# SciML/NeuralPDE.jl

Hardware: NVIDIA H100
Metric: collocation-points/sec (loss+grad) (higher is better)
Workload: dtype f32

## Files before the change

neuralpde.jl_b200/csrc/tc_kernel.cu:

```cuda
#include "tc_common.cuh"

namespace pinn {

using Fp = FpBlock<kTcW>;

struct CtaShared : CtaBase {
  int split, off_Q;
  uint8_t* stash;
  TcNetSmem nets[PINN_MAX_NETS];
};

struct LoopCtx {
  uint32_t fp;
  uint32_t bt;
  uint32_t tP;
  uint32_t tQ;
  float* gb;
  float* gw;
  uint32_t taddr;
  int act, split, p, lane, g0, g1, flag;
  __device__ __forceinline__ LoopCtx(uint32_t fp_, uint32_t bt_, uint32_t tP_, uint32_t tQ_, const Tid& t, int act_, int ng,
                                     int flag_, int split_ = 0, float* gb_ = nullptr, float* gw_ = nullptr)
      : fp(fp_), bt(bt_), tP(tP_), tQ(tQ_), gb(gb_), gw(gw_), taddr(t.lane_addr), act(act_), split(split_), p(t.p), lane(t.lane),
        g0(t.hh * (ng / kNH)), g1((t.hh + 1) * (ng / kNH)), flag(flag_) {}
};

template <int N1, int N2, bool PURE, int AK>
__device__ __forceinline__ void l0_fwd_loop(const LoopCtx lc, const PassInfo<N1, N2> pi, const float* xp, float* up) {
  constexpr int C = 1 + N1 + N2;
  float x[PINN_MAX_IN], u[C];
#pragma unroll
  for (int k = 0; k < PINN_MAX_IN; ++k) x[k] = xp[k];
#pragma unroll
  for (int c = 0; c < C; ++c) u[c] = up[c];
#pragma unroll 1
  for (int g = lc.g0; g < lc.g1; ++g) {
    float h[C][GW];
#pragma unroll
    for (int i = 0; i < GW; i += 2) {
      float za[C], zb2[C];
      first_layer_elem<kTcW>(lc.fp, pi, x, g * GW + i, za);
      first_layer_elem<kTcW>(lc.fp, pi, x, g * GW + i + 1, zb2);
      P2 zz[C], hv[C];
#pragma unroll
      for (int c = 0; c < C; ++c) zz[c] = mk2(za[c], zb2[c]);
      chain_fwd<N1, N2, PURE, AK, P2>(lc.act, pi.ch, zz, hv);
#pragma unroll
      for (int c = 0; c < C; ++c) { h[c][i] = hv[c].v.x; h[c][i + 1] = hv[c].v.y; }
      if (lc.flag) {
        const float w0 = lds_f32(lc.fp + (Fp::WL + g * GW + i) * 4), w1 = lds_f32(lc.fp + (Fp::WL + g * GW + i + 1) * 4);
#pragma unroll
        for (int c = 0; c < C; ++c) u[c] = fmaf(w1, hv[c].v.y, fmaf(w0, hv[c].v.x, u[c]));
      }
    }
#pragma unroll
    for (int c = 0; c < C; ++c) store_half(lc.tP + c * kTileBytes, lc.tQ + c * kTileBytes, lc.p, g * GW, h[c], lc.split != 0);
  }
#pragma unroll
  for (int c = 0; c < C; ++c) up[c] = u[c];
}

template <int C, int NK, bool SPLIT>
__device__ __forceinline__ void fwd_mma(float (&d)[C][16], uint32_t sP, uint32_t sQ, uint32_t whi, uint32_t wlo) {
  const int wg = threadIdx.x >> 7;
  const uint32_t aoff = (wg & 1) * 8192u, boff = (wg >> 1) * 32u * 128u;
  const uint64_t dwhi = tc::make_desc(whi + boff, 0, 1024), dwlo = tc::make_desc(wlo + boff, 0, 1024);
  tc::wgmma_fence();
#pragma unroll
  for (int c = 0; c < C; ++c) {
    const uint64_t dahi = tc::make_desc(sP + c * kTileBytes + aoff, 0, 1024);
    const uint64_t dalo = tc::make_desc(sQ + c * kTileBytes + aoff, 0, 1024);
#pragma unroll
    for (int pr = 0; pr < (SPLIT ? 3 : 1); ++pr) {
      const uint64_t a = (pr == 2) ? dalo : dahi, b = (pr == 1) ? dwlo : dwhi;
#pragma unroll
      for (int k = 0; k < NK; ++k)
        tc::wgmma_n32<0, 0>(d[c], a + 2 * k, b + 2 * k, (pr | k) ? 1u : 0u);
    }
  }
  tc::wgmma_commit();
  tc::wgmma_wait0();
}
template <int C>
__device__ __forceinline__ void fwd_mma_any(float (&d)[C][16], uint32_t sP, uint32_t sQ, uint32_t whi, uint32_t wlo, int nk,
                                            bool split) {
  switch (nk * 2 + (split ? 1 : 0)) {
    case 2: fwd_mma<C, 1, false>(d, sP, sQ, whi, wlo); break;
    case 3: fwd_mma<C, 1, true>(d, sP, sQ, whi, wlo); break;
    case 4: fwd_mma<C, 2, false>(d, sP, sQ, whi, wlo); break;
    case 5: fwd_mma<C, 2, true>(d, sP, sQ, whi, wlo); break;
    case 6: fwd_mma<C, 3, false>(d, sP, sQ, whi, wlo); break;
    case 7: fwd_mma<C, 3, true>(d, sP, sQ, whi, wlo); break;
    case 8: fwd_mma<C, 4, false>(d, sP, sQ, whi, wlo); break;
    default: fwd_mma<C, 4, true>(d, sP, sQ, whi, wlo); break;
  }
}

template <int N1, int N2, bool PURE, int AK, int C>
__device__ __forceinline__ void tl_fwd_frag(const float (&d)[C][16], const LoopCtx lc, const Chan<N1, N2> ch, float* scratch) {
  const int wg = threadIdx.x >> 7, w = (threadIdx.x >> 5) & 3;
  const int row0 = 64 * (wg & 1) + 16 * w + (lc.lane >> 2);
  const int col0 = 32 * (wg >> 1) + 2 * (lc.lane & 3);
  float u[2][C];
#pragma unroll
  for (int r = 0; r < 2; ++r)
#pragma unroll
    for (int c = 0; c < C; ++c) u[r][c] = 0.f;
#pragma unroll
  for (int i = 0; i < 16; i += 2) {
    const int rh = (i >> 1) & 1;
    const int row = row0 + 8 * rh, col = col0 + 8 * (i >> 2);
    P2 zz[C], hv[C];
    zz[0] = mk2(d[0][i] + lds_f32(lc.bt + col * 4), d[0][i + 1] + lds_f32(lc.bt + (col + 1) * 4));
#pragma unroll
    for (int c = 1; c < C; ++c) zz[c] = mk2(d[c][i], d[c][i + 1]);
    chain_fwd<N1, N2, PURE, AK, P2>(lc.act, ch, zz, hv);
    const uint32_t off = tc::swz_off(row, col);
#pragma unroll
    for (int c = 0; c < C; ++c) {
      const uint32_t hx = tc::pack_bf16(hv[c].v.x, hv[c].v.y);
      asm volatile("st.shared.b32 [%0], %1;" ::"r"(lc.tP + c * kTileBytes + off), "r"(hx) : "memory");
      if (lc.split)
        asm volatile("st.shared.b32 [%0], %1;" ::"r"(lc.tQ + c * kTileBytes + off), "r"(bf16x2_lo(hv[c].v.x, hv[c].v.y, hx))
                     : "memory");
    }
    if (lc.flag) {
      const float w0 = lds_f32(lc.fp + (Fp::WL + col) * 4), w1 = lds_f32(lc.fp + (Fp::WL + col + 1) * 4);
#pragma unroll
      for (int c = 0; c < C; ++c) u[rh][c] = fmaf(w1, hv[c].v.y, fmaf(w0, hv[c].v.x, u[rh][c]));
    }
  }
  if (lc.flag) {
#pragma unroll
    for (int r = 0; r < 2; ++r)
#pragma unroll
      for (int c = 0; c < C; ++c) {
        float s = u[r][c];
        s += __shfl_xor_sync(0xffffffffu, s, 1);
        s += __shfl_xor_sync(0xffffffffu, s, 2);
        if ((lc.lane & 3) == 0) atomicAdd(&scratch[c * kTcPts + row0 + 8 * r], s);
      }
  }
}

template <int C, int NKO>
__device__ __forceinline__ void dgrad_mma(float (&d)[C][16], uint32_t sP, uint32_t whi) {
  const uint32_t poff = (threadIdx.x >> 7) * 32u * 128u;
  const uint64_t dw = tc::make_desc(whi, 0, 1024);
  tc::wgmma_fence();
#pragma unroll
  for (int c = 0; c < C; ++c) {
    const uint64_t dz = tc::make_desc(sP + c * kTileBytes + poff, 0, 1024);
#pragma unroll
    for (int k = 0; k < NKO; ++k)
      tc::wgmma_n32<1, 0>(d[c], dw + 128 * k, dz + 2 * k, k ? 1u : 0u);
  }
  tc::wgmma_commit();
  tc::wgmma_wait0();
}
template <int C>
__device__ __forceinline__ void dgrad_mma_any(float (&d)[C][16], uint32_t sP, uint32_t whi, int nko) {
  switch (nko) {
    case 1: dgrad_mma<C, 1>(d, sP, whi); break;
    case 2: dgrad_mma<C, 2>(d, sP, whi); break;
    case 3: dgrad_mma<C, 3>(d, sP, whi); break;
    default: dgrad_mma<C, 4>(d, sP, whi); break;
  }
}
template <int C>
__device__ __forceinline__ void wgrad_mma(float (&dw)[32], float (&db)[8], uint32_t sP, uint32_t sQ, uint32_t s_ones) {
  const uint32_t poff = (threadIdx.x >> 7) * 32u * 128u;
  const uint64_t d1 = tc::make_desc(s_ones, 0, 0);
  tc::wgmma_fence();
#pragma unroll
  for (int c = 0; c < C; ++c) {
    const uint64_t dh = tc::make_desc(sQ + c * kTileBytes + poff, 0, 1024), dz = tc::make_desc(sP + c * kTileBytes + poff, 0, 1024);
#pragma unroll
    for (int k = 0; k < 2; ++k) tc::wgmma_n64<1, 1>(dw, dh + 128 * k, dz + 128 * k, (c | k) ? 1u : 0u);
  }
  const uint64_t dz0 = tc::make_desc(sP + poff, 0, 1024);
#pragma unroll
  for (int k = 0; k < 2; ++k) tc::wgmma_n16<1, 1>(db, dz0 + 128 * k, d1, k ? 1u : 0u);
  tc::wgmma_commit();
  tc::wgmma_wait0();
}

template <int NF>
__device__ __forceinline__ void frag_store_rows(float* base, int ld, const float (&d)[NF]) {
  const int w = (threadIdx.x >> 5) & 3, lane = threadIdx.x & 31;
  const bool odd = (lane & 1) != 0;
  float* row = base + (16 * w + (lane >> 2) + (odd ? 8 : 0)) * ld + 4 * ((lane >> 1) & 1);
#pragma unroll
  for (int j = 0; j < NF / 4; ++j) {
    const float r0 = __shfl_xor_sync(0xffffffffu, odd ? d[4 * j] : d[4 * j + 2], 1);
    const float r1 = __shfl_xor_sync(0xffffffffu, odd ? d[4 * j + 1] : d[4 * j + 3], 1);
    *reinterpret_cast<float4*>(row + 8 * j) =
        odd ? make_float4(r0, r1, d[4 * j + 2], d[4 * j + 3]) : make_float4(d[4 * j], d[4 * j + 1], r0, r1);
  }
}

template <int N1, int N2, bool PURE, int AK, int C>
__device__ __forceinline__ void tl_bwd_frag(const float (&d)[C][16], const LoopCtx lc, const Chan<N1, N2> ch, const float* ubs) {
  const int wg = threadIdx.x >> 7, w = (threadIdx.x >> 5) & 3;
  const int row0 = 64 * (wg & 1) + 16 * w + (lc.lane >> 2);
  const int col0 = 32 * (wg >> 1) + 2 * (lc.lane & 3);
  const float* hbar = tc::s_acc + TM_X * kAccRows;
#pragma unroll
  for (int i = 0; i < 16; i += 2) {
    const int row = row0 + 8 * ((i >> 1) & 1), col = col0 + 8 * (i >> 2);
    P2 zz[C], hv[C], zv[C];
    zz[0] = mk2(d[0][i] + lds_f32(lc.bt + col * 4), d[0][i + 1] + lds_f32(lc.bt + (col + 1) * 4));
#pragma unroll
    for (int c = 1; c < C; ++c) zz[c] = mk2(d[c][i], d[c][i + 1]);
    if (lc.flag) {
      const float w0 = lds_f32(lc.fp + (Fp::WL + col) * 4), w1 = lds_f32(lc.fp + (Fp::WL + col + 1) * 4);
#pragma unroll
      for (int c = 0; c < C; ++c) {
        const float u = ubs[c * kTcPts + row];
        hv[c] = mk2(w0 * u, w1 * u);
      }
    } else {
#pragma unroll
      for (int c = 0; c < C; ++c) hv[c] = mk2(hbar[(c * 64 + col) * kAccRows + row], hbar[(c * 64 + col + 1) * kAccRows + row]);
    }
    chain_bwd<N1, N2, PURE, AK, P2>(lc.act, ch, zz, hv, zv);
    const uint32_t off = tc::swz_off(row, col);
#pragma unroll
    for (int c = 0; c < C; ++c)
      asm volatile("st.shared.b32 [%0], %1;" ::"r"(lc.tP + c * kTileBytes + off), "r"(tc::pack_bf16(zv[c].v.x, zv[c].v.y))
                   : "memory");
  }
}

template <int N1, int N2, bool PURE, int AK>
__device__ __forceinline__ void l0_bwd_store_loop(const LoopCtx lc, const PassInfo<N1, N2> pi, const float* xp) {
  constexpr int C = 1 + N1 + N2;
  float x[PINN_MAX_IN];
#pragma unroll
  for (int k = 0; k < PINN_MAX_IN; ++k) x[k] = xp[k];
#pragma unroll 1
  for (int g = lc.g0; g < lc.g1; ++g) {
    float hb[C][GWB];
#pragma unroll
    for (int c = 0; c < C; ++c) acc_ldg(lc.taddr + TM_X + c * 64 + g * GWB, hb[c]);
#pragma unroll
    for (int i = 0; i < GWB; i += 2) {
      float za[C], zb2[C];
      first_layer_elem<kTcW>(lc.fp, pi, x, g * GWB + i, za);
      first_layer_elem<kTcW>(lc.fp, pi, x, g * GWB + i + 1, zb2);
      P2 zz[C], hv[C], zv[C];
#pragma unroll
      for (int c = 0; c < C; ++c) { zz[c] = mk2(za[c], zb2[c]); hv[c] = mk2(hb[c][i], hb[c][i + 1]); }
      chain_bwd<N1, N2, PURE, AK, P2>(lc.act, pi.ch, zz, hv, zv);
#pragma unroll
      for (int c = 0; c <= N1; ++c) { hb[c][i] = zv[c].v.x; hb[c][i + 1] = zv[c].v.y; }
    }
#pragma unroll
    for (int c = 0; c <= N1; ++c) store_half(lc.tP + c * kTileBytes, lc.tP, lc.p, g * GWB, hb[c], false);
  }
}

template <int N1, int N2, bool PURE, int AK>
__device__ __forceinline__ void l0_bwd_loop(const LoopCtx lc, const PassInfo<N1, N2> pi, const float* xp, const float* ubp) {
  constexpr int C = 1 + N1 + N2;
  float x[PINN_MAX_IN], ub[C];
#pragma unroll
  for (int k = 0; k < PINN_MAX_IN; ++k) x[k] = xp[k];
#pragma unroll
  for (int c = 0; c < C; ++c) ub[c] = ubp[c];
  const int re = reduceg_elem(lc.lane);
  const bool rlead = reduceg_lead(lc.lane);
  const int n1w = pi.n1w;
#pragma unroll 1
  for (int g = lc.g0; g < lc.g1; ++g) {
    float hb[C][GW];
    if (!lc.flag) {
#pragma unroll
      for (int c = 0; c < C; ++c) acc_ldg(lc.taddr + TM_X + c * 64 + g * GW, hb[c]);
    } else {
#pragma unroll
      for (int i = 0; i < GW; ++i) {
        const float wl = lds_f32(lc.fp + (Fp::WL + g * GW + i) * 4);
#pragma unroll
        for (int c = 0; c < C; ++c) hb[c][i] = wl * ub[c];
      }
    }
    float zv0[GW], zvd[N1 > 0 ? N1 : 1][GW];
#pragma unroll
    for (int i = 0; i < GW; ++i) {
      float zz[C], hv[C], zv[C];
      first_layer_elem<kTcW>(lc.fp, pi, x, g * GW + i, zz);
#pragma unroll
      for (int c = 0; c < C; ++c) hv[c] = hb[c][i];
      chain_bwd<N1, N2, PURE, AK, float>(lc.act, pi.ch, zz, hv, zv);
      zv0[i] = zv[0];
#pragma unroll
      for (int jd = 0; jd < N1; ++jd) zvd[jd][i] = zv[1 + jd];
    }
    const float bs = warp_reduceg(zv0, lc.lane);
    if (rlead) atomicAdd(lc.gb + g * GW + re, bs);
#pragma unroll
    for (int k = 0; k < PINN_MAX_IN; ++k) {
      if (k < pi.d_in) {
        float gk[GW];
#pragma unroll
        for (int i = 0; i < GW; ++i) {
          float gg = zv0[i] * x[k];
#pragma unroll
          for (int jd = 0; jd < N1; ++jd) gg += (pi.dir1[jd] == k) ? zvd[jd][i] : 0.f;
          gk[i] = gg;
        }
        const float gs = warp_reduceg(gk, lc.lane);
        if (rlead) atomicAdd(lc.gw + g * GW + re + (long long)n1w * k, gs);
      }
    }
  }
}

template <int N1, int N2, bool PURE, int AK>
__device__ __noinline__ uint32_t net_forward(CtaShared* cs, const DevProblem* Pp, const DevTerm* tmp, int slot,
                                             int want_grad, uint32_t phase) {
  extern __shared__ __align__(1024) uint8_t smem[];
  constexpr int C = 1 + N1 + N2;
  const DevTerm& tm = *tmp;
  const int net_id = tm.used_net[slot];
  const DevNet& net = Pp->nets[net_id];
  const DevChan& dc = tm.chan[slot];
  const TcNetSmem ns = cs->nets[net_id];
  const float* fp = reinterpret_cast<const float*>(smem + ns.fp);
  uint8_t* tP = smem + cs->off_P;
  uint8_t* tQ = smem + cs->off_Q;
  const Misc ms = misc_of(smem + cs->off_misc, cs->mx_dim, cs->mx_taps);
  const uint32_t accm = 0;
  const bool split = cs->split != 0;
  PassInfo<N1, N2> pi;
  load_pass<N1, N2>(pi, net, dc);
  const int TL = pi.TL;
  const Tid t = tid_of();
  const int tid = t.tid, p = t.p;
  float x[PINN_MAX_IN];
#pragma unroll
  for (int k = 0; k < PINN_MAX_IN; ++k) x[k] = (k < pi.d_in) ? ms.Xs[dc.rows[k] * kTcPts + p] : 0.f;
  uint8_t* stash_slot = cs->stash + (size_t)slot * cs->tl_max * kTcMaxC * kTileBytes;

  dbg_mark(cs, 10);
  float u[C];
#pragma unroll
  for (int c = 0; c < C; ++c) u[c] = 0.f;
  if (tid < C * kTcPts / 4) reinterpret_cast<float4*>(ms.scratch)[tid] = make_float4(0.f, 0.f, 0.f, 0.f);
  {
    const LoopCtx lc(tc::smem_u32(fp), tc::smem_u32(fp), tc::smem_u32(tP), tc::smem_u32(tQ), t, net.acts[0], pi.n1w / GW, TL == 0, split);
    l0_fwd_loop<N1, N2, PURE, AK>(lc, pi, x, u);
  }
  for (int l = 1; l <= TL; ++l) {
    const int n_in = net.dims[l], n_out = net.dims[l + 1];
    const int act = net.acts[l];
    tc::fence_async_smem();
    __syncthreads();
    dbg_mark(cs, 11);
    if (want_grad && tid == 0) {
      for (int c = 0; c < C; ++c)
        tc::bulk_store(stash_slot + (size_t)(l - 1) * kTcMaxC * kTileBytes + (size_t)c * kTileBytes, tP + c * kTileBytes, kTileBytes);
      tc::bulk_commit();
    }
    float d[C][16];
    {
      const uint32_t sP = tc::smem_u32(tP), sQ = tc::smem_u32(tQ);
      const uint32_t whi = tc::smem_u32(smem + ns.w_hi[l - 1]), wlo = tc::smem_u32(smem + ns.w_lo[l - 1]);
      const int nk = n_in / 16;
      fwd_mma_any<C>(d, sP, sQ, whi, wlo, nk, split);
    }
    dbg_mark(cs, 13);
    if (want_grad && tid == 0) tc::bulk_wait_read0();
    __syncthreads();
    dbg_mark(cs, 14);
    const LoopCtx lc(tc::smem_u32(fp), tc::smem_u32(fp) + (Fp::BT + (l - 1) * 64) * 4, tc::smem_u32(tP), tc::smem_u32(tQ), t, act, 0, l == TL, split);
    tl_fwd_frag<N1, N2, PURE, AK, C>(d, lc, pi.ch, ms.scratch);
  }
  finish_forward<C>(cs, tm, slot, ms, fp + Fp::BL, t, u);
  return phase;
}

template <int N1, int N2, bool PURE, int AK>
__device__ __noinline__ uint32_t net_backward(CtaShared* cs, const DevProblem* Pp, const DevTerm* tmp, int slot,
                                              uint32_t phase) {
  extern __shared__ __align__(1024) uint8_t smem[];
  constexpr int C = 1 + N1 + N2;
  const DevTerm& tm = *tmp;
  const int net_id = tm.used_net[slot];
  const DevNet& net = Pp->nets[net_id];
  const DevChan& dc = tm.chan[slot];
  const TcNetSmem ns = cs->nets[net_id];
  const float* fp = reinterpret_cast<const float*>(smem + ns.fp);
  uint8_t* tP = smem + cs->off_P;
  uint8_t* tQ = smem + cs->off_Q;
  const Misc ms = misc_of(smem + cs->off_misc, cs->mx_dim, cs->mx_taps);
  const uint32_t accm = 0;
  float* partial = cs->partial;
  PassInfo<N1, N2> pi;
  load_pass<N1, N2>(pi, net, dc);
  const int L = pi.L, TL = pi.TL;
  const Tid t = tid_of();
  const int tid = t.tid, p = t.p;
  uint32_t ld_phase = (phase >> 1) & 1u;
  float x[PINN_MAX_IN];
#pragma unroll
  for (int k = 0; k < PINN_MAX_IN; ++k) x[k] = (k < pi.d_in) ? ms.Xs[dc.rows[k] * kTcPts + p] : 0.f;
  uint8_t* stash_slot = cs->stash + (size_t)slot * cs->tl_max * kTcMaxC * kTileBytes;

  dbg_mark(cs, 20);
  float ub[C];
  gather_ubar<C>(tm, slot, ms, p, ub);
  if (t.hh == 0) {
#pragma unroll
    for (int c = 0; c < C; ++c) ms.scratch[c * kTcPts + p] = ub[c];
  }
  last_layer_grad<C>(t, ub, pi.nL, partial + net.w_off[L - 1], partial + net.b_off[L - 1], tc::smem_u32(tQ), tc::smem_u32(tP),
                     kTileBytes, 0u, accm + TM_Y, kTcW);

  const uint32_t sP = tc::smem_u32(tP), sQ = tc::smem_u32(tQ);
  const int wg = tid >> 7;
  float* hand = tc::s_acc + TM_X * kAccRows;
  float* wpart = reinterpret_cast<float*>(tP);
  float* bpart = ms.scratch;
  static_assert(4 * 64 <= kTcMaxC * kTcPts, "the bias partials fit ms.scratch");
  for (int l = TL; l >= 1; --l) {
    const int n_in = net.dims[l], n_out = net.dims[l + 1];
    const int act = net.acts[l];
    float* gb = partial + net.b_off[l];
    float* gw = partial + net.w_off[l];
    const float* bt = fp + Fp::BT + (l - 1) * 64;
    const uint32_t whi = tc::smem_u32(smem + ns.w_hi[l - 1]);
    dbg_mark(cs, 21);
    if (tid == 0 && l == TL) {
      const uint8_t* src = stash_slot + (size_t)(l - 1) * kTcMaxC * kTileBytes;
      tc::mbar_arrive_expect_tx(ms.bar_ld, C * kTileBytes);
      for (int c = 0; c < C; ++c) tc::bulk_load(tQ + c * kTileBytes, src + (size_t)c * kTileBytes, kTileBytes, ms.bar_ld);
    }
    wait_bar(ms.bar_ld, ld_phase);
    dbg_mark(cs, 22);
    {
      float d[C][16];
      fwd_mma_any<C>(d, sQ, sQ, whi, whi, n_in / 16, false);
      __syncthreads();
      dbg_mark(cs, 24);
      const LoopCtx lc(tc::smem_u32(fp), tc::smem_u32(bt), sP, sQ, t, act, 0, l == TL);
      tl_bwd_frag<N1, N2, PURE, AK, C>(d, lc, pi.ch, ms.scratch);
    }
    tc::fence_async_smem();
    __syncthreads();
    dbg_mark(cs, 26);
    {
      float d[C][16];
      dgrad_mma_any<C>(d, sP, whi, n_out / 16);
#pragma unroll
      for (int c = 0; c < C; ++c) frag_store_rows(hand + c * 64 * kAccRows + 32 * wg, kAccRows, d[c]);
    }
    dbg_mark(cs, 27);
    {
      float dw[32], db[8];
      wgrad_mma<C>(dw, db, sP, sQ, tc::smem_u32(smem + cs->off_ones));
      __syncthreads();
      if (tid == 0 && l > 1) {
        const uint8_t* src = stash_slot + (size_t)(l - 2) * kTcMaxC * kTileBytes;
        tc::mbar_arrive_expect_tx(ms.bar_ld, C * kTileBytes);
        for (int c = 0; c < C; ++c) tc::bulk_load(tQ + c * kTileBytes, src + (size_t)c * kTileBytes, kTileBytes, ms.bar_ld);
      }
      frag_store_rows(wpart + wg * 64 * 64, 64, dw);
      if ((t.lane & 3) == 0) {
        const int o = 16 * (t.warp & 3) + (t.lane >> 2);
        bpart[wg * 64 + o] = db[0];
        bpart[wg * 64 + o + 8] = db[2];
      }
    }
    __syncthreads();
    dbg_mark(cs, 28);
#pragma unroll 1
    for (int e = tid; e < 64 * 64; e += kTcThreads) {
      const int k = e >> 6, o = e & 63;
      if (k < n_in && o < n_out) atomicAdd(gw + o + (long long)n_out * k, ((wpart[e] + wpart[4096 + e]) + wpart[8192 + e]) + wpart[12288 + e]);
    }
    if (tid < n_out) atomicAdd(gb + tid, ((bpart[tid] + bpart[64 + tid]) + bpart[128 + tid]) + bpart[192 + tid]);
  }

  {
    __syncthreads();
    dbg_mark(cs, 29);
    const int act0 = net.acts[0];
    float* gb0 = partial + net.b_off[0];
    float* gw0 = partial + net.w_off[0];
    if (TL == 0) {
      const LoopCtx lc(tc::smem_u32(fp), tc::smem_u32(fp), sP, sQ, t, act0, pi.n1w / GW, 1, 0, gb0, gw0);
      l0_bwd_loop<N1, N2, PURE, AK>(lc, pi, x, ub);
    } else {
      coord_tiles<N1>(t, sQ, x, pi.dir1, N2 > 0);
      const LoopCtx lc(tc::smem_u32(fp), tc::smem_u32(fp), sP, sQ, t, act0, pi.n1w / GWB, 0);
      l0_bwd_store_loop<N1, N2, PURE, AK>(lc, pi, x);
      layer0_grad<N1>(t, sP, kTileBytes, 0u, sQ, N2 > 0, accm + TM_Y, kTcW, pi.n1w, pi.d_in, gw0, gb0);
    }
  }
  __syncthreads();
  dbg_mark(cs, 30);
  return (ld_phase << 1) | (phase & 1u);
}


__global__ void __launch_bounds__(kTcThreads, 1) tc_loss_grad_kernel(const __grid_constant__ TcArgs args) {
  extern __shared__ __align__(1024) uint8_t smem[];
  __shared__ CtaShared cs;
  const int tid = threadIdx.x;
  const DevProblem* Pp = args.prob;
  const DevProblem& P = *Pp;
  const Misc ms = misc_of(smem + args.off_misc, args.mx_dim, args.mx_taps);
  float* partial = args.partial + (long long)blockIdx.x * args.partial_stride;
  const bool want_grad = (args.mode == 0);
  const float* theta = args.theta;
  const DbgSpan span = dbg_span_begin(args.dbg);

  for (long long i = (long long)tid * 32; i < args.n_theta; i += (long long)kTcThreads * 32) tc::prefetch_l2(theta + i);
  {
    const char* nets0 = reinterpret_cast<const char*>(&Pp->nets[0]);
    const char* terms0 = reinterpret_cast<const char*>(&Pp->terms[0]);
    const int nb_nets = args.n_nets * (int)sizeof(DevNet), nb_terms = args.n_terms * (int)sizeof(DevTerm);
    if (tid == 0) tc::prefetch_l2(Pp);
    for (int o = tid * 128; o < nb_nets; o += kTcThreads * 128) tc::prefetch_l2(nets0 + o);
    for (int o = tid * 128; o < nb_terms; o += kTcThreads * 128) tc::prefetch_l2(terms0 + o);
    const int tile = args.tile_begin + (int)blockIdx.x;
    if (tile < args.tile_end && tid < 32) {
      int ti = 0;
      while (ti + 1 < args.n_terms && tile >= args.dyn[ti + 1].tile0) ++ti;
      const long long p0 = (long long)(tile - args.dyn[ti].tile0) * kTcPts;
      const long long row_bytes = 4ll * args.term_dim[ti];
      const long long off = p0 * row_bytes + (long long)tid * 128;
      if (off < args.dyn[ti].n * row_bytes) tc::prefetch_l2(reinterpret_cast<const char*>(args.dyn[ti].pts) + off);
    }
  }
  if (tid == 0) {
    tc::mbar_init(ms.bar_ld, 1);
    tc::fence_barrier_init();
    cs.split = args.split; cs.off_Q = args.off_Q;
    cs.stash = args.stash + (long long)blockIdx.x * args.stash_per_cta;
    for (int k = 0; k < PINN_MAX_NETS; ++k) cs.nets[k] = args.nets[k];
    cta_base_init(cs, args, partial);
  }
  if (tid == 0) tc::s_acc = args.acc + (size_t)blockIdx.x * kAccCols * kAccRows;
  cta_setup(args, ms, partial, P.n_theta, want_grad);
  for (int kn = 0; kn < P.n_nets; ++kn) {
    const DevNet& net = P.nets[kn];
    const TcNetSmem& ns = args.nets[kn];
    if (ns.fp < 0) continue;
    stage_fp_block<kTcW>(reinterpret_cast<float*>(smem + ns.fp), net, theta);
    const int L = net.n_layers;
    {
      constexpr int kItMax = kTcMaxTL * 512 / kTcThreads;
      const int n_items = (L - 2) * 512;
      float w[kItMax][8];
#pragma unroll
      for (int it = 0; it < kItMax; ++it) {
        const int i = tid + it * kTcThreads;
        if (i < n_items) {
          const int l = 1 + i / 512, r = i & 511;
          const int o = r & 63, kc = r >> 6;
          const int n_in = net.dims[l], n_out = net.dims[l + 1];
          const long long woff = net.w_off[l];
#pragma unroll
          for (int e = 0; e < 8; ++e) {
            const int k = kc * 8 + e;
            w[it][e] = (o < n_out && k < n_in) ? __ldg(&theta[woff + o + (long long)n_out * k]) : 0.f;
          }
        }
      }
#pragma unroll
      for (int it = 0; it < kItMax; ++it) {
        const int i = tid + it * kTcThreads;
        if (i < n_items) {
          const int l = 1 + i / 512, r = i & 511;
          const int o = r & 63, kc = r >> 6;
          uint8_t* thi = smem + ns.w_hi[l - 1];
          uint8_t* tlo = smem + ns.w_lo[l - 1];
          const float* v = w[it];
          uint32_t h[4];
#pragma unroll
          for (int e = 0; e < 4; ++e) h[e] = tc::pack_bf16(v[2 * e], v[2 * e + 1]);
          *reinterpret_cast<uint4*>(thi + tc::swz_chunk(o, kc)) = make_uint4(h[0], h[1], h[2], h[3]);
          if (args.split)
            *reinterpret_cast<uint4*>(tlo + tc::swz_chunk(o, kc)) = make_uint4(
                bf16x2_lo(v[0], v[1], h[0]), bf16x2_lo(v[2], v[3], h[1]), bf16x2_lo(v[4], v[5], h[2]), bf16x2_lo(v[6], v[7], h[3]));
        }
      }
    }
  }
  tc::fence_async_smem();
  __syncthreads();
  dbg_mark(&cs, 2);
  uint32_t phase = 0;

  for (int tile = args.tile_begin + blockIdx.x; tile < args.tile_end; tile += gridDim.x) {
    if (tid >= 128 && tid < 128 + (int)((sizeof(DevNet) * PINN_MAX_NETS + 127) / 128))
      tc::prefetch_l1(reinterpret_cast<const char*>(&P.nets[0]) + (tid - 128) * 128);
    uint32_t ldp = (phase >> 1) & 1u;
    const TileRef tr = stage_tile(args, P, ms, tile, ldp);
    phase = (phase & 1u) | (ldp << 1);
    const DevTerm* tmp = &P.terms[tr.ti];
    const DevTerm& tm = *tmp;
    const int n_used = tm.n_used;
    dbg_mark(&cs, 3);

    for (int slot = 0; slot < n_used; ++slot) {
      const int k1 = tm.chan[slot].n1, k2 = tm.chan[slot].n2, pu = tm.chan[slot].pure;
      const int ak = args.net_ak[tm.used_net[slot]];
      PINN_TC_DISPATCH(kTcMaxC, k1, k2, pu, ak, (phase = net_forward<A1, A2, PU, AK>(&cs, Pp, tmp, slot, want_grad ? 1 : 0, phase)));
    }

    dbg_mark(&cs, 4);
    residual_step(args, P, tm, ms, tr, smem + args.off_Q, (size_t)args.off_Q_bytes, partial, want_grad);

    dbg_mark(&cs, 5);
    if (want_grad) {
      if (tid == 0) tc::bulk_wait0();
      __syncthreads();
      dbg_mark(&cs, 6);
      for (int slot = n_used - 1; slot >= 0; --slot) {
        const int k1 = tm.chan[slot].n1, k2 = tm.chan[slot].n2, pu = tm.chan[slot].pure;
        const int ak = args.net_ak[tm.used_net[slot]];
        if (n_used > 1) {
          PINN_TC_DISPATCH(kTcMaxC, k1, k2, pu, ak, (phase = net_forward<A1, A2, PU, AK>(&cs, Pp, tmp, slot, 0, phase)));
        }
        PINN_TC_DISPATCH(kTcMaxC, k1, k2, pu, ak, (phase = net_backward<A1, A2, PU, AK>(&cs, Pp, tmp, slot, phase)));
      }
    }
  }

  __syncthreads();
  dbg_mark(&cs, 7);
  cta_finish(args, cs, span, ms, P, want_grad);
}

size_t tc_misc_bytes(int mx_dim, int mx_taps) {
  return (size_t)mx_dim * kTcPts * 4 + 2 * (size_t)mx_taps * kTcPts * 4 + (size_t)kTcMaxC * kTcPts * 4 + kTcPts * 4 +
         PINN_MAX_TERMS * 8 + 16 + 16;
}

cudaError_t tc_launch(const TcArgs& a, int grid, size_t smem, cudaStream_t st) {
  return launch_fused_kernel<tc_loss_grad_kernel>(a, grid, kTcThreads, smem, st);
}

}
```

Baseline: 94.15 million.

## Compute last-layer and layer-0 weight grads with wgmma, drop atomics for plain RMW

Replaces the previous last-layer and layer-0 gradient helpers with wgmma-based reductions over staged bf16 tiles. Per-warpgroup partials go through shared memory and are summed once per block. The per-layer atomicAdd loops on the block-private partial buffer become plain load-add-store, and L2 prefetches for the gradient slices are issued ahead of the updates. This removes atomic traffic and scalar reduction work, at the cost of extra __syncthreads, more shared-memory staging, and bf16 rounding of ub in the last-layer product.

New measurement: 96.44 million (median of 6 runs). Within noise of the previous version (+2.4%).

```diff
diff --git a/neuralpde.jl_b200/csrc/tc_kernel.cu b/neuralpde.jl_b200/csrc/tc_kernel.cu
--- a/neuralpde.jl_b200/csrc/tc_kernel.cu
+++ b/neuralpde.jl_b200/csrc/tc_kernel.cu
@@ -185,6 +185,54 @@
   tc::wgmma_wait0();
 }
 
+template <int C>
+__device__ __forceinline__ void last_grad_mma(float (&d)[8], uint32_t sH, uint32_t sU) {
+  const uint32_t poff = (threadIdx.x >> 7) * 32u * 128u;
+  tc::wgmma_fence();
+#pragma unroll
+  for (int c = 0; c < C; ++c) {
+    const uint64_t dh = tc::make_desc(sH + c * kTileBytes + poff, 0, 1024), du = tc::make_desc(sU + c * kTileBytes + poff, 0, 1024);
+#pragma unroll
+    for (int k = 0; k < 2; ++k) tc::wgmma_n16<1, 1>(d, dh + 128 * k, du + 128 * k, (c | k) ? 1u : 0u);
+  }
+  tc::wgmma_commit();
+  tc::wgmma_wait0();
+}
+template <int C>
+__device__ __noinline__ void last_grad_part(uint32_t sH, uint32_t sU, float* lpart) {
+  float d[8];
+  last_grad_mma<C>(d, sH, sU);
+  __syncthreads();
+  const int lane = threadIdx.x & 31, wg = threadIdx.x >> 7;
+  if ((lane & 3) == 0) {
+    const int o = 16 * ((threadIdx.x >> 5) & 3) + (lane >> 2);
+    lpart[wg * 64 + o] = d[0] + d[1];
+    lpart[wg * 64 + o + 8] = d[2] + d[3];
+  }
+}
+template <int N1, bool XLO>
+__device__ __forceinline__ void l0_grad_mma(float (&d)[8], uint32_t sZ, uint32_t sB) {
+  const uint32_t poff = (threadIdx.x >> 7) * 32u * 128u;
+  const uint64_t dz0 = tc::make_desc(sZ + poff, 0, 1024);
+  tc::wgmma_fence();
+#pragma unroll
+  for (int k = 0; k < 2; ++k) tc::wgmma_n16<1, 1>(d, dz0 + 128 * k, tc::make_desc(sB + poff, 0, 1024) + 128 * k, k ? 1u : 0u);
+  if (XLO) {
+    const uint64_t dlo = tc::make_desc(sB + (1 + N1) * kTileBytes + poff, 0, 1024);
+#pragma unroll
+    for (int k = 0; k < 2; ++k) tc::wgmma_n16<1, 1>(d, dz0 + 128 * k, dlo + 128 * k, 1u);
+  }
+#pragma unroll
+  for (int j = 0; j < N1; ++j) {
+    const uint64_t dz = tc::make_desc(sZ + (1 + j) * kTileBytes + poff, 0, 1024);
+    const uint64_t de = tc::make_desc(sB + (1 + j) * kTileBytes + poff, 0, 1024);
+#pragma unroll
+    for (int k = 0; k < 2; ++k) tc::wgmma_n16<1, 1>(d, dz + 128 * k, de + 128 * k, 1u);
+  }
+  tc::wgmma_commit();
+  tc::wgmma_wait0();
+}
+
 template <int NF>
 __device__ __forceinline__ void frag_store_rows(float* base, int ld, const float (&d)[NF]) {
   const int w = (threadIdx.x >> 5) & 3, lane = threadIdx.x & 31;
@@ -331,7 +379,6 @@
   uint8_t* tP = smem + cs->off_P;
   uint8_t* tQ = smem + cs->off_Q;
   const Misc ms = misc_of(smem + cs->off_misc, cs->mx_dim, cs->mx_taps);
-  const uint32_t accm = 0;
   const bool split = cs->split != 0;
   PassInfo<N1, N2> pi;
   load_pass<N1, N2>(pi, net, dc);
@@ -395,7 +442,6 @@
   uint8_t* tP = smem + cs->off_P;
   uint8_t* tQ = smem + cs->off_Q;
   const Misc ms = misc_of(smem + cs->off_misc, cs->mx_dim, cs->mx_taps);
-  const uint32_t accm = 0;
   float* partial = cs->partial;
   PassInfo<N1, N2> pi;
   load_pass<N1, N2>(pi, net, dc);
@@ -407,19 +453,37 @@
 #pragma unroll
   for (int k = 0; k < PINN_MAX_IN; ++k) x[k] = (k < pi.d_in) ? ms.Xs[dc.rows[k] * kTcPts + p] : 0.f;
   uint8_t* stash_slot = cs->stash + (size_t)slot * cs->tl_max * kTcMaxC * kTileBytes;
+  const uint32_t sP = tc::smem_u32(tP), sQ = tc::smem_u32(tQ);
+  const int wg = tid >> 7;
 
   dbg_mark(cs, 20);
+  if (tid < 3) tc::prefetch_l2(partial + net.w_off[L - 1] + 31 * tid);
+  if (tid == 3) tc::prefetch_l2(partial + net.b_off[L - 1]);
   float ub[C];
   gather_ubar<C>(tm, slot, ms, p, ub);
-  if (t.hh == 0) {
-#pragma unroll
-    for (int c = 0; c < C; ++c) ms.scratch[c * kTcPts + p] = ub[c];
-  }
-  last_layer_grad<C>(t, ub, pi.nL, partial + net.w_off[L - 1], partial + net.b_off[L - 1], tc::smem_u32(tQ), tc::smem_u32(tP),
-                     kTileBytes, 0u, accm + TM_Y, kTcW);
-
-  const uint32_t sP = tc::smem_u32(tP), sQ = tc::smem_u32(tQ);
-  const int wg = tid >> 7;
+  {
+    float bs = 0.f;
+    if (t.hh == 0) {
+      bs = warp_sum<float>(ub[0]);
+#pragma unroll
+      for (int c = 0; c < C; ++c) {
+        ms.scratch[c * kTcPts + p] = ub[c];
+        const uint32_t hi = tc::pack_bf16(ub[c], 0.f);
+        const uint32_t u = sQ + c * kTileBytes;
+        sts_v4(u + tc::swz_chunk(p, 0), hi | (bf16x2_lo(ub[c], 0.f, hi) << 16), 0u, 0u, 0u);
+        sts_v4(u + tc::swz_chunk(p, 1), 0u, 0u, 0u, 0u);
+      }
+    }
+    tc::fence_async_smem();
+    __syncthreads();
+    float* lpart = reinterpret_cast<float*>(tP);
+    last_grad_part<C>(sP, sQ, lpart);
+    if (t.hh == 0 && t.lane == 0) lpart[256 + t.warp] = bs;
+    __syncthreads();
+    if (tid < pi.nL) partial[net.w_off[L - 1] + tid] += ((lpart[tid] + lpart[64 + tid]) + lpart[128 + tid]) + lpart[192 + tid];
+    if (tid == kTcThreads - 1) partial[net.b_off[L - 1]] += ((lpart[256] + lpart[257]) + lpart[258]) + lpart[259];
+  }
+
   float* hand = tc::s_acc + TM_X * kAccRows;
   float* wpart = reinterpret_cast<float*>(tP);
   float* bpart = ms.scratch;
@@ -457,6 +521,8 @@
       for (int c = 0; c < C; ++c) frag_store_rows(hand + c * 64 * kAccRows + 32 * wg, kAccRows, d[c]);
     }
     dbg_mark(cs, 27);
+    if (tid <= n_in * n_out / 32) tc::prefetch_l2(gw + 32 * tid);
+    if (tid == kTcThreads - 1) tc::prefetch_l2(gb);
     {
       float dw[32], db[8];
       wgrad_mma<C>(dw, db, sP, sQ, tc::smem_u32(smem + cs->off_ones));
@@ -475,12 +541,23 @@
     }
     __syncthreads();
     dbg_mark(cs, 28);
-#pragma unroll 1
-    for (int e = tid; e < 64 * 64; e += kTcThreads) {
-      const int k = e >> 6, o = e & 63;
-      if (k < n_in && o < n_out) atomicAdd(gw + o + (long long)n_out * k, ((wpart[e] + wpart[4096 + e]) + wpart[8192 + e]) + wpart[12288 + e]);
-    }
-    if (tid < n_out) atomicAdd(gb + tid, ((bpart[tid] + bpart[64 + tid]) + bpart[128 + tid]) + bpart[192 + tid]);
+    {
+      constexpr int kE = 64 * 64 / kTcThreads;
+      float g[kE], s[kE];
+#pragma unroll
+      for (int i = 0; i < kE; ++i) {
+        const int e = tid + i * kTcThreads, k = e >> 6, o = e & 63;
+        g[i] = (k < n_in && o < n_out) ? gw[o + n_out * k] : 0.f;
+        s[i] = ((wpart[e] + wpart[4096 + e]) + wpart[8192 + e]) + wpart[12288 + e];
+      }
+      const float gbv = tid < n_out ? gb[tid] : 0.f;
+#pragma unroll
+      for (int i = 0; i < kE; ++i) {
+        const int e = tid + i * kTcThreads, k = e >> 6, o = e & 63;
+        if (k < n_in && o < n_out) gw[o + n_out * k] = g[i] + s[i];
+      }
+      if (tid < n_out) gb[tid] = gbv + (((bpart[tid] + bpart[64 + tid]) + bpart[128 + tid]) + bpart[192 + tid]);
+    }
   }
 
   {
@@ -493,10 +570,29 @@
       const LoopCtx lc(tc::smem_u32(fp), tc::smem_u32(fp), sP, sQ, t, act0, pi.n1w / GW, 1, 0, gb0, gw0);
       l0_bwd_loop<N1, N2, PURE, AK>(lc, pi, x, ub);
     } else {
+      if (tid <= pi.n1w * pi.d_in / 32) tc::prefetch_l2(gw0 + 32 * tid);
+      if (tid == kTcThreads - 1) tc::prefetch_l2(gb0);
       coord_tiles<N1>(t, sQ, x, pi.dir1, N2 > 0);
       const LoopCtx lc(tc::smem_u32(fp), tc::smem_u32(fp), sP, sQ, t, act0, pi.n1w / GWB, 0);
       l0_bwd_store_loop<N1, N2, PURE, AK>(lc, pi, x);
-      layer0_grad<N1>(t, sP, kTileBytes, 0u, sQ, N2 > 0, accm + TM_Y, kTcW, pi.n1w, pi.d_in, gw0, gb0);
+      tc::fence_async_smem();
+      __syncthreads();
+      float d[8];
+      l0_grad_mma<N1, (N2 > 0)>(d, sP, sQ);
+      __syncthreads();
+      float* part = reinterpret_cast<float*>(tP);
+      frag_store_rows(part + wg * 64 * 16, 16, d);
+      __syncthreads();
+      const int n1w = pi.n1w, d_in = pi.d_in;
+      static_assert(PINN_MAX_IN <= 8, "column 8 of the layer-0 product is the bias");
+#pragma unroll 1
+      for (int e = tid; e < 9 * 64; e += kTcThreads) {
+        const int k = e >> 6, o = e & 63;
+        const float* q = part + o * 16 + k;
+        const float s = ((q[0] + q[1024]) + q[2048]) + q[3072];
+        if (o < n1w && k < d_in) gw0[o + n1w * k] += s;
+        if (o < n1w && k == 8) gb0[o] += s;
+      }
     }
   }
   __syncthreads();
```
